# tjjones6/Computational-Fluid-Dynamics

Measured on AMD Instinct MI355X. Metric: Poisson MLUPS + steps/sec, cavity 4096² @1/2/4/8 GPU; % HBM roofline, higher is better.
Workload: dtype f64

## Files before the change

### computational-fluid-dynamics_amd/csrc/internal.hpp

```cpp
#pragma once

#include <stdexcept>
#include <string>
#include <vector>

#include "../../include/cfd_amd.h"

namespace cfd {

struct Error : std::runtime_error {
  int code;
  Error(int c, const std::string& m) : std::runtime_error(m), code(c) {}
};

void set_last_error(const std::string& msg);

struct LoopHub;
struct LoopOp {
  int kind;
  double* buf;
  size_t count;
  int peer;
};

// ... 1 lines not shown
  void* nccl = nullptr;
  int nranks = 1, rank = 0, device = 0;
  LoopHub* hub = nullptr;
  std::vector<LoopOp> pending;
  void* ev_ready = nullptr;
  void* ev_done = nullptr;
  double* tmp = nullptr;
  size_t tmp_count = 0;
};

void comm_unique_id(unsigned char* id_out);
Comm* comm_init(const unsigned char* id, int nranks, int rank, int device);
LoopHub* loop_hub_create(int nranks);
void loop_hub_destroy(LoopHub* h);
Comm* comm_init_loopback(LoopHub* h, int rank, int device);
void comm_destroy(Comm* c);
void comm_info(Comm* c, int* nranks, int* rank, int* transport);
void comm_group_start(Comm* c);
void comm_group_end(Comm* c, void* stream);
void comm_send(Comm* c, const double* buf, size_t count, int peer, void* stream);
void comm_recv(Comm* c, double* buf, size_t count, int peer, void* stream);
void comm_halo_exchange(Comm* c, const double* send_lo, double* recv_lo, int peer_lo, const double* send_hi,
                        double* recv_hi, int peer_hi, size_t count, void* stream);
long long comm_exchange_check(Comm* c, int peer, size_t count);
void comm_allreduce_max(Comm* c, double* buf, size_t count, void* stream);
void comm_allreduce_sum(Comm* c, double* buf, size_t count, void* stream);

void write_vtk_arrays(const cfd_params& p, const std::string& filename, double time_value, const double* uc,
                      const double* vc, const double* pr, const double* temp = nullptr);
void write_pvd(const std::string& filename, const char* const* files, const double* times, int n);

bool host_is_fluid(const cfd_params& p, int j, int i);

}
```

### computational-fluid-dynamics_amd/csrc/lexw.hpp

```cpp
#pragma once

#include "kernels.hpp"

namespace cfd {

constexpr int LEXW_SHARDS = 8;
#ifndef CFD_LEXW_RAMP_EDGE_FULL
#define CFD_LEXW_RAMP_EDGE_FULL 1
#endif
#ifndef CFD_LEXW_W2
#define CFD_LEXW_W2 2
#endif
#ifndef CFD_LEXW_W3
#define CFD_LEXW_W3 2
#endif
#define CFD_LEXW_MIN_WAVES(NS) ((NS) <= 2 ? CFD_LEXW_W2 : CFD_LEXW_W3)

__host__ __device__ constexpr int lexw_twc(int ns) { return ns >= 5 ? 106 : ns == 4 ? 110 : PAIR_TWC; }
__host__ __device__ constexpr int lexw_ch(int ns) { return ns >= 5 ? 10 : 8; }

constexpr int LEXW_RAMP_BANDS = 256;
struct LexRamp {
  int nb, th, row0;
  int wsplit;
  int xa, xn, xreach;
  unsigned band[LEXW_RAMP_BANDS];
};

__host__ __device__ inline int lexw_ramp_waves(const LexRamp& rp, int ctiles, int b, int ca, int cb, int o,
                                               int* ctile, int* half) {
  int sp[4], n = 0;
  if (rp.wsplit && ca == 0 && cb >= ca) sp[n++] = 0;
  if (rp.xn > 0 && rp.row0 + (b + 1) * rp.th + rp.xreach >= 0)
    for (int c = max(rp.xa, ca); c <= min(rp.xa + rp.xn - 1, cb); ++c)
      if (c != 0 && c != ctiles - 1) sp[n++] = c;
  if (rp.wsplit && cb == ctiles - 1 && cb > 0) sp[n++] = cb;
  int extra = 0;
  for (int q = 0; q < n; ++q) {
    const int at = sp[q] - ca + extra;
    if (o < at) break;
    if (o == at || o == at + 1) {
      *ctile = sp[q];
      *half = o - at;
      return n;
    }
    ++extra;
  }
  *ctile = ca + o - extra;
  *half = -1;
  return n;
}

// ... 21 lines not shown
}
__global__ void lexw_bits_scatter_kernel(LexCtl L, int ka, int kb, const double* __restrict__ flags) {
  const int k = ka + (int)(blockIdx.x * blockDim.x + threadIdx.x);
  if (k > kb || !(flags[k - ka] > 0.0)) return;
  const int q = L.kmax + k;
  atomicOr(L.bits + (q >> 6), 1ull << (q & 63));
}

__device__ __forceinline__ bool lexw_go_on(const LexCtl& L, int ka, int kb, bool first_wave, int lane) {
  if (L.stop[0] != 0) return false;
  const double tol = L.tol[0];
  for (int k = ka; k <= kb; ++k) {
    const bool go = (k == 0) ? (L.tol[1] > tol) : lexw_slot_exceeds(L, k);
    if (!go) {
      if (first_wave && lane == 0) {
        L.stop[1] = k;
        L.stop[0] = (k == 0 || k >= L.kexact) ? 1 : 2;
      }
      return false;
    }
  }
  return true;
}

#define LX_SLOT(X) ((((ROT) + 4 - (X)) % 5 + 10) % 5)
#define LX_S10(X) ((((6 * (ROT) + 5 * (PAR)) % 10 + 9 - (X)) % 10 + 20) % 10)


struct LxDefer {
  double xp, ps;
  int k;
};

template <int NS>
struct LexRun {
  double2 w[NS][5];
  double2 fr[10];
  double2 np[5];
  double2 nf[5];
  unsigned long long mask;
  LxDefer d;
};

struct LexCtx {
  int H0;
  int K;
  double tol;
  double o2, o3, o4;
  int jg, jr1;
  double gz;
};

__device__ __forceinline__ double2 lx_ld(const WaveCtx<CAVITY>& x, const double* base, int R) {
  const int Rc = min(max(R, x.rmin), x.rmax);
  return *reinterpret_cast<const double2*>(base + (size_t)(Rc - x.g.row_lo) * (size_t)x.g.pitch + x.gic);
}

constexpr int LX_ACT = 1;
#ifndef CFD_LEXW_GROUPS
#define CFD_LEXW_GROUPS 1
#endif
#ifndef CFD_LEXW_ALLRC
#define CFD_LEXW_ALLRC 0
#endif
constexpr int LX_SAMPLE = 2;
struct LxAct {
  bool a, b, c;
  bool a2, b2;
  unsigned u;
};
// ... 257 lines not shown
    if constexpr ((MODE & LX_ACT) != 0) ex = ex && act.c;
  } else {
    const double pc = m.x;
    double pW = dpp_from_left(old.y);
    if constexpr (STEP) pW = (rs == 2 && cc.sa == 2 && x.gi == x.c.step_i + 1) ? 0.0 + pc : pW;
    const double pS = row1 ? pc : sb.x;
    const double pE = m.y;
    ex = fabs(residual_at<CASE>(x.c, 0, 0, 0, 0, pc, pW, pE, pS, nb.x, fc.x)) > thr;
    if constexpr (EDGE) ex = ex && cc.ka == 3;
    if constexpr (STEP) {
      ex = ex && (rs == 0 || cc.sa == 2);
      if (rowc && cc.sa == 1) {
        ex = false;
        bool on = true;
        if constexpr ((MODE & LX_ACT) != 0) on = act.b;
        if (FULL && on) {
          d.xp = (pE - 2.0 * pc + pW) * x.c.idx2;
          d.ps = pS;
          d.k = (Hh - 1 - c0k) / 2 + 1;
          if (LASTH && x.out_lane && rrow) {
            L.cscr[0] = d.xp;
            L.cscr[1] = d.ps;
            L.cscr[2] = (double)d.k;
          }
        }
      }
    }
    if constexpr ((MODE & LX_ACT) != 0) ex = ex && act.b;
  }
  exi = ex ? 1 : exi;
  asm volatile("" : "+v"(exi));
}

template <int MODE, int T, int X>
constexpr bool lx_res_row() { return !(MODE & LX_SAMPLE) || T == X; }

template <int CASE>
struct LxCols {
  LxCol cc[2];
  LxoCol oc;
};

template <int CASE, int S, int NS, int T, int ROT, int PAR, int MODE, bool EDGE, bool RC, bool UP = false>
__device__ __forceinline__ void lx_sweeps(const WaveCtx<CAVITY>& x, const LexCtx& lc, const LexCtl& L,
                                          const LxCols<CASE>& cl, LexRun<NS>& s, int R, const LxAct& act, int& exi) {
  if constexpr (S < NS) {
    constexpr int D = UP ? -1 : 1;
    if constexpr (CASE == CAVITY) {
      lx_row<ROT, PAR ^ 1, 0, MODE, EDGE, false, lx_res_row<MODE, T, 2 * S + 1>(), UP>(
          x, lc, cl.cc, s.w[S], R + D * (2 * S + 1), 2 * S + 1, act, s.fr[LX_S10(2 * S + 1)], exi);
      lx_row<ROT, PAR, 1, MODE, EDGE, S == NS - 1, lx_res_row<MODE, T, 2 * S + 2>(), UP>(
          x, lc, cl.cc, s.w[S], R + D * (2 * S + 2), 2 * S + 2, act, s.fr[LX_S10(2 * S + 2)], exi);
    } else {
      lxo_row<CASE, ROT, PAR ^ 1, 0, MODE, EDGE, RC, false, lx_res_row<MODE, T, 2 * S + 1>(), S == 0, false, UP>(
          x, lc, L, cl.oc, s.w[S], R + D * (2 * S + 1), 2 * S + 1, act, s.fr[LX_S10(2 * S + 1)], exi, s.d);
      double2* nxt = nullptr;
      if constexpr (S + 1 < NS && !UP) nxt = &s.w[S + 1][LX_SLOT(2 * S + 3)];
      lxo_row<CASE, ROT, PAR, 1, MODE, EDGE, RC, S == NS - 1, lx_res_row<MODE, T, 2 * S + 2>(), false, S == NS - 1, UP>(
          x, lc, L, cl.oc, s.w[S], R + D * (2 * S + 2), 2 * S + 2, act, s.fr[LX_S10(2 * S + 2)], exi, s.d, nxt);
    }
    if constexpr (S + 1 < NS) s.w[S + 1][LX_SLOT(2 * S + 2)] = s.w[S][LX_SLOT(2 * S + 2)];
    lx_sweeps<CASE, S + 1, NS, T, ROT, PAR, MODE, EDGE, RC, UP>(x, lc, L, cl, s, R, act, exi);
  }
}

template <int CASE, int NS, int T, int ROT, int PAR, int MODE, bool EDGE, bool RC, bool UP = false>
__device__ __forceinline__ void lx_step(const WaveCtx<CAVITY>& x, const LexCtx& lc, const LexCtl& L,
                                        const LxCols<CASE>& cl, LexRun<NS>& s, int R, unsigned long long bit) {
  constexpr int D = UP ? -1 : 1;
  s.w[0][LX_SLOT(0)] = s.np[LX_SLOT(0)];
  s.fr[LX_S10(1)] = s.nf[LX_SLOT(0)];
  s.np[LX_SLOT(-4)] = lx_ld(x, x.pin, R - 4 * D);
  s.nf[LX_SLOT(-4)] = lx_ld(x, x.f, R - 3 * D);
  int exi = 0;
  const LxAct act = lx_act<MODE, CASE == BACKSTEP && EDGE && RC>(lc, x.gi, R);
  lx_sweeps<CASE, 0, NS, T, ROT, PAR, MODE, EDGE, RC, UP>(x, lc, L, cl, s, R, act, exi);
  if constexpr (UP) return;
  if constexpr ((MODE & LX_SAMPLE) && (T < 1 || T > 2 * NS)) return;
  s.mask |= exi ? bit : 0ull;
}

__device__ __forceinline__ unsigned long long wave_or64(unsigned long long v) {
#pragma unroll
  for (int off = 32; off > 0; off >>= 1) {
    const unsigned lo = (unsigned)v, hi = (unsigned)(v >> 32);
    v |= (unsigned long long)(unsigned)__shfl_xor((int)lo, off, 64) |
         ((unsigned long long)(unsigned)__shfl_xor((int)hi, off, 64) << 32);
  }
  return v;
}

__device__ __forceinline__ void lexw_flush(const LexCtl& L, int sh, int q0, const unsigned long long (&b)[3], int len) {
  unsigned long long* G = L.bits + (size_t)sh * L.words;
#pragma unroll
  for (int c = 0; c < 3; ++c) {
    if (c * 64 >= len || b[c] == 0) continue;
    const int q = q0 + c * 64;
    const int w = q >> 6, o = q & 63;
    if (w < L.words) atomicOr(&G[w], b[c] << o);
    if (o && w + 1 < L.words) atomicOr(&G[w + 1], b[c] >> (64 - o));
  }
}

template <int CASE, int NS, int MODE, bool EDGE, bool RC = false, bool UP = false>
__device__ __forceinline__ void lx_march(const WaveCtx<CAVITY>& x, const LexCtx& lc, const LexCtl& L, int y0, int y1,
                                         int c0, int lane, int shard) {
  static_assert(!UP || (!(MODE & LX_ACT) && !EDGE && !RC), "upward march: the unmasked, unchecked interior bands");
  constexpr int H = 2 * NS + 1;
  constexpr int D = UP ? -1 : 1;
  const int Rb0 = UP ? y0 - H : y1 - 1 + H;
  const int Rbeg = UP ? Rb0 - (Rb0 & 1) : Rb0 + (Rb0 & 1);
  const int nsteps = (y1 - y0) + 2 * H + (Rb0 & 1);
  LexRun<NS> s;
  const double2 z = make_double2(0.0, 0.0);
#pragma unroll
  for (int k = 0; k < 5; ++k)
#pragma unroll
    for (int q = 0; q < NS; ++q) s.w[q][k] = z;
#pragma unroll
  for (int k = 0; k < 10; ++k) s.fr[k] = z;
  {
    constexpr int ROT = 0;
#pragma unroll
    for (int q = 0; q < 4; ++q) {
      s.np[LX_SLOT(-q)] = lx_ld(x, x.pin, Rbeg - D * q);
      s.nf[LX_SLOT(-q)] = lx_ld(x, x.f, Rbeg - D * (q - 1));
    }
  }
  s.mask = 0ull;
  s.d = LxDefer{0.0, 0.0, -1};
  LxCols<CASE> cl;
  if constexpr (EDGE && CASE == CAVITY) cl.cc[0] = lx_col(x, x.gi), cl.cc[1] = lx_col(x, x.gi + 1);
  if constexpr (EDGE && CASE != CAVITY)
    cl.oc = LxoCol{lxo_kind(x, x.gi), lxo_kind(x, x.gi + 1), lxs_class(x, x.gi), lxs_class(x, x.gi + 1)};
  int R = Rbeg;
  if constexpr (UP) {
    for (int st = 0; st < nsteps; st += 10, R += 10) {
      lx_step<CASE, NS, 0, 0, 0, MODE, EDGE, RC, true>(x, lc, L, cl, s, R, 0ull);
      lx_step<CASE, NS, 1, 1, 1, MODE, EDGE, RC, true>(x, lc, L, cl, s, R + 1, 0ull);
      lx_step<CASE, NS, 2, 2, 0, MODE, EDGE, RC, true>(x, lc, L, cl, s, R + 2, 0ull);
      lx_step<CASE, NS, 3, 3, 1, MODE, EDGE, RC, true>(x, lc, L, cl, s, R + 3, 0ull);
      lx_step<CASE, NS, 4, 4, 0, MODE, EDGE, RC, true>(x, lc, L, cl, s, R + 4, 0ull);
      lx_step<CASE, NS, 5, 0, 1, MODE, EDGE, RC, true>(x, lc, L, cl, s, R + 5, 0ull);
      lx_step<CASE, NS, 6, 1, 0, MODE, EDGE, RC, true>(x, lc, L, cl, s, R + 6, 0ull);
      lx_step<CASE, NS, 7, 2, 1, MODE, EDGE, RC, true>(x, lc, L, cl, s, R + 7, 0ull);
      lx_step<CASE, NS, 8, 3, 0, MODE, EDGE, RC, true>(x, lc, L, cl, s, R + 8, 0ull);
      lx_step<CASE, NS, 9, 4, 1, MODE, EDGE, RC, true>(x, lc, L, cl, s, R + 9, 0ull);
    }
    return;
  }
#define LX_BIT(T) ((((st + (T)) >> 1) < 64) ? (1ull << ((st + (T)) >> 1)) : 0ull)
  for (int st = 0; st < nsteps; st += 10, R -= 10) {
#if CFD_LEXW_GROUPS
    if constexpr (RC && !EDGE && CASE == CHANNEL) {
      if (R - 8 >= 2 && R - 8 > x.rmin && R + 2 * NS < lc.jg && R + 2 * NS < x.rmax) {
        lx_step<CASE, NS, 0, 0, 0, MODE, EDGE, false>(x, lc, L, cl, s, R, LX_BIT(0));
        lx_step<CASE, NS, 1, 1, 1, MODE, EDGE, false>(x, lc, L, cl, s, R - 1, LX_BIT(1));
        lx_step<CASE, NS, 2, 2, 0, MODE, EDGE, false>(x, lc, L, cl, s, R - 2, LX_BIT(2));
        lx_step<CASE, NS, 3, 3, 1, MODE, EDGE, false>(x, lc, L, cl, s, R - 3, LX_BIT(3));
        lx_step<CASE, NS, 4, 4, 0, MODE, EDGE, false>(x, lc, L, cl, s, R - 4, LX_BIT(4));
        lx_step<CASE, NS, 5, 0, 1, MODE, EDGE, false>(x, lc, L, cl, s, R - 5, LX_BIT(5));
        lx_step<CASE, NS, 6, 1, 0, MODE, EDGE, false>(x, lc, L, cl, s, R - 6, LX_BIT(6));
        lx_step<CASE, NS, 7, 2, 1, MODE, EDGE, false>(x, lc, L, cl, s, R - 7, LX_BIT(7));
        lx_step<CASE, NS, 8, 3, 0, MODE, EDGE, false>(x, lc, L, cl, s, R - 8, LX_BIT(8));
        lx_step<CASE, NS, 9, 4, 1, MODE, EDGE, false>(x, lc, L, cl, s, R - 9, LX_BIT(9));
        continue;
      }
    }
#endif
    lx_step<CASE, NS, 0, 0, 0, MODE, EDGE, RC>(x, lc, L, cl, s, R, LX_BIT(0));
    lx_step<CASE, NS, 1, 1, 1, MODE, EDGE, RC>(x, lc, L, cl, s, R - 1, LX_BIT(1));
    lx_step<CASE, NS, 2, 2, 0, MODE, EDGE, RC>(x, lc, L, cl, s, R - 2, LX_BIT(2));
    lx_step<CASE, NS, 3, 3, 1, MODE, EDGE, RC>(x, lc, L, cl, s, R - 3, LX_BIT(3));
    lx_step<CASE, NS, 4, 4, 0, MODE, EDGE, RC>(x, lc, L, cl, s, R - 4, LX_BIT(4));
    lx_step<CASE, NS, 5, 0, 1, MODE, EDGE, RC>(x, lc, L, cl, s, R - 5, LX_BIT(5));
    lx_step<CASE, NS, 6, 1, 0, MODE, EDGE, RC>(x, lc, L, cl, s, R - 6, LX_BIT(6));
    lx_step<CASE, NS, 7, 2, 1, MODE, EDGE, RC>(x, lc, L, cl, s, R - 7, LX_BIT(7));
    lx_step<CASE, NS, 8, 3, 0, MODE, EDGE, RC>(x, lc, L, cl, s, R - 8, LX_BIT(8));
    lx_step<CASE, NS, 9, 4, 1, MODE, EDGE, RC>(x, lc, L, cl, s, R - 9, LX_BIT(9));
  }
#undef LX_BIT
  const unsigned long long m = x.out_lane ? s.mask : 0ull;
  const int sh = 63 - lane;
  const unsigned long long lo = m << sh, hi = sh ? (m >> (64 - sh)) : 0ull;
  unsigned long long b[3] = {wave_or64(lo), wave_or64(hi), 0ull};
  const int Bd0 = (lc.H0 - c0 - Rbeg - 2) / 2 + 1;
  if (lane == 0) lexw_flush(L, shard, Bd0 - 63 + L.kmax, b, 128);
}

__host__ __device__ inline void lexw_rows(const Geo& g, int H0, int K, int ns, int ct, int* lo, int* hi,
                                          bool open = false) {
  const int twc = lexw_twc(ns);
  if (!open) {
    const int cmin = max(ct * twc, 1), cmax = min(ct * twc + twc - 1, g.nx);
    *lo = max(g.j0, H0 - 2 * ns - 2 * (K - 1) - cmax);
    *hi = min(g.j1, H0 + 2 * ns - 1 - cmin);
  } else {
    const int cmin = max(ct * twc, 0), cmax = min(ct * twc + twc - 1, g.nx + 1);
    *lo = max(g.wj0, H0 - 2 * ns - 2 * (K - 1) - cmax - 2);
    *hi = min(g.wj1, H0 + 2 * ns - 1 - cmin);
  }
}

#ifndef CFD_LEXW_STAMPS
#define CFD_LEXW_STAMPS 0
#endif
#if CFD_LEXW_STAMPS
constexpr int LEXW_STAMP_LAUNCHES = 8192;
static __device__ unsigned long long lexw_stamp_buf[LEXW_STAMP_LAUNCHES * 8 * 3];
#ifndef LEXW_WSTAMP_L0
#define LEXW_WSTAMP_L0 1500
#endif
// ... 268 lines not shown
```

### computational-fluid-dynamics_amd/csrc/params.cpp

```cpp
#include <algorithm>
#include <cmath>
#include <cstring>
#include <string>

#include "internal.hpp"
#include "mg.hpp"

namespace {

double omega_2d(int nx, int ny) {
  const double pi = 3.14159265358979323846;
  const double rho_j = 0.5 * (std::cos(pi / (nx + 1)) + std::cos(pi / (ny + 1)));
  const double denom = 1.0 + std::sqrt(std::max(1e-14, 1.0 - rho_j * rho_j));
  return 2.0 / denom;
}

}

extern "C" int cfd_params_init(int case_id, double re, int nx, int ny, double dt, cfd_params* out) {
  if (!out) {
    cfd::set_last_error("null output");
    return CFD_E_ARG;
  }
  cfd_params p;
// ... 116 lines not shown

extern "C" int cfd_tuning_default(const cfd_params* p, int knob, int* value) {
  if (!p || !value) {
    cfd::set_last_error("null argument");
    return CFD_E_ARG;
  }
  const bool cav = p->case_id == CFD_CAVITY || p->case_id == CFD_RAYLEIGH_BENARD;
  switch (knob) {
    case CFD_TUNE_LEXW_EDGE_PCT: *value = p->ny <= 2048 ? 75 : 100; return CFD_OK;
    case CFD_TUNE_PAIR_EDGE_PCT: *value = cav ? 80 : 45; return CFD_OK;
    case CFD_TUNE_MARCH_MIN_TH: *value = (p->case_id == CFD_CHANNEL || p->ordering == CFD_ORDER_LEX) ? 16 : 24; return CFD_OK;
    case CFD_TUNE_TENT_TH: *value = 64; return CFD_OK;
    case CFD_TUNE_LEXW_RAMP_PCT:
      *value = p->case_id == CFD_BACKSTEP ? 100 : 0;
      return CFD_OK;
    case CFD_TUNE_TILE_ROUNDS: *value = cav ? 1 : 0; return CFD_OK;
    case CFD_TUNE_MARCH_ORDER: *value = 0; return CFD_OK;
    case CFD_TUNE_LEXW_LEFT: *value = 1; return CFD_OK;
    case CFD_TUNE_LEXW_UPDOWN: *value = 1; return CFD_OK;
    case CFD_TUNE_RESIDENT:
      *value = (cav || p->case_id == CFD_CHANNEL) ? 1 : 0;
      return CFD_OK;
    case CFD_TUNE_PAIR_WPS:
    case CFD_TUNE_WAVE_WPS:
    case CFD_TUNE_LEXW_WAVES:
      cfd::set_last_error("this knob's default is derived from the device's occupancy at cfd_create");
      return CFD_E_STATE;
    default:
      cfd::set_last_error("unknown tuning knob");
      return CFD_E_ARG;
  }
}

bool cfd::mg_make_plan(const cfd_params& p, MgPlan& plan, std::string& why) {
  if (p.case_id != CFD_CAVITY && p.case_id != CFD_RAYLEIGH_BENARD) {
    why = "multigrid covers the cavity and Rayleigh-Benard (case rule): the channel and the step keep SOR";
    return false;
  }
  if (p.nx < 2 || p.ny < 2 || !(p.dx > 0)) {
    why = "multigrid needs a grid of at least 2 x 2 cells and dx > 0 (grid rule)";
    return false;
  }
  int nx = p.nx, ny = p.ny, n = 0;
  plan = MgPlan{};
  for (;;) {
    MgLevel& L = plan.lv[n];
    L.nx = nx;
    L.ny = ny;
    L.pitch = ((nx + 3) + 15) / 16 * 16;
    L.lds_p = L.lds_f = -1;
    const int m = std::max(nx, ny);
    L.coarse_sweeps = 4 * m;
    L.h2 = std::ldexp(1.0, 2 * n) * (p.dx * p.dx);
    L.ih2 = 1.0 / L.h2;
    const double d = 0.5 + std::ldexp(1.0, -(n + 1));
    L.cS = 1.0 / d;
    L.g = 1.0 - L.cS;
    const double pi = 3.14159265358979323846;
    const double omega = 2.0 / (1.0 + std::sin(pi / (m + 1)));
    L.one_m_omega = 1.0 - omega;
    for (int k = 0; k < 16; ++k) {
      const double ew = k & 1, ee = (k >> 1) & 1, en = (k >> 2) & 1, cs = (k & 8) ? L.cS : 1.0;
      L.rdiag[k] = 1.0 / (((ew + ee) + en) + cs);
      L.omr[k] = omega * L.rdiag[k];
    }
    ++n;
// ... 51 lines not shown
```

### computational-fluid-dynamics_amd/csrc/solver.hip

```cpp
#include <algorithm>
#include <cmath>
#include <cstdlib>
#include <cstring>
#include <string>
#include <vector>

#include "internal.hpp"
#include "kernels.hpp"
#include "lexw.hpp"
#include "small.hpp"
#include "tile.hpp"
#include "resident.hpp"
#include "open.hpp"
#include "smlex.hpp"
#include "seqsum.hpp"
#include "mg.hpp"

#ifndef CFD_LEXW_WALL_SPLIT
#define CFD_LEXW_WALL_SPLIT 1
#endif

namespace cfd {

static thread_local std::string g_last_error;
// ... 180 lines not shown
      case CFD_TUNE_PAIR_WPS: resident_pair_waves = std::max(1, std::min(v, 4)) * 4 * n_cu; break;
      case CFD_TUNE_WAVE_WPS: resident_waves = std::max(1, std::min(v, 4)) * 4 * n_cu; break;
      case CFD_TUNE_LEXW_WAVES: resident_lexw_waves = std::max(64, v); break;
      case CFD_TUNE_LEXW_EDGE_PCT: lexw_edge_pct = std::max(10, std::min(100, v)); break;
      case CFD_TUNE_PAIR_EDGE_PCT: pair_edge_pct = std::max(10, std::min(100, v)); break;
      case CFD_TUNE_MARCH_MIN_TH: march_min_th = std::max(1, v); break;
      case CFD_TUNE_TENT_TH: tent_th = std::max(4, v); break;
      case CFD_TUNE_LEXW_RAMP_PCT: lexw_ramp_pct = std::max(0, std::min(100, v)); break;
      case CFD_TUNE_TILE_ROUNDS: tile_rounds = std::max(0, std::min(v, 16)); break;
      case CFD_TUNE_MARCH_ORDER: march_flags = (march_flags & ~8) | (v ? 8 : 0); break;
      case CFD_TUNE_LEXW_LEFT: lexw_left = v != 0; break;
      case CFD_TUNE_RESIDENT: res_knob = v != 0; break;
      case CFD_TUNE_LEXW_UPDOWN: lexw_updown = v != 0; break;
      default: throw Error(CFD_E_ARG, "unknown tuning knob");
    }
  }

  unsigned long long* lexbits = nullptr;
  size_t lexbits_words = 0;
  double* resmax = nullptr;
  hipEvent_t ev_f0 = nullptr, ev_f1 = nullptr;
  int resident_lexw_waves = 2048;
  int lexw_edge_pct = 100;
  int lexw_ramp_pct = 0;
  bool lexw_left = true;
  bool lexw_updown = true;
  bool step_lexw_ok() const { return P.step_i >= 2 && P.inlet_jmax >= 1 && P.inlet_jmax <= P.ny - 2; }
  bool use_lexw() const {
    return P.ordering == CFD_ORDER_LEX &&
           (P.case_id == CFD_CAVITY || P.case_id == CFD_CHANNEL || (P.case_id == CFD_BACKSTEP && step_lexw_ok()));
  }
  double* cscr = nullptr;
  int lexw_ns() const {
    const int ns = (P.case_id != CFD_CAVITY || P.sweeps_per_launch < 1) ? 4 : P.sweeps_per_launch;
    return multi() ? std::min(ns, 3) : ns;
  }
  bool ranks() const { return comm && comm->nranks > 1; }
  static constexpr int LEXW_RED_EVERY = 8;
  double* lexflags = nullptr;
  size_t lexflags_n = 0;
  void lexw_reduce_bits(const LexCtl& L, int ka, int kb) {
    if (!ranks() || ka > kb) return;
    const int n = kb - ka + 1;
    if ((size_t)n > lexflags_n) throw Error(CFD_E_STATE, "lexicographic ordering: bit reduction range");
    lexw_bits_gather_kernel<<<(n + 255) / 256, 256, 0, st>>>(L, ka, kb, lexflags);
    check_launch("lexw_bits_gather");
    comm_allreduce_max(comm, lexflags, (size_t)n, st);
    lexw_bits_scatter_kernel<<<(n + 255) / 256, 256, 0, st>>>(L, ka, kb, lexflags);
    check_launch("lexw_bits_scatter");
  }
  void seq_sum(const Strip& s, const double* a, const double* b, int mode, double* acc, bool accumulate) {
    T.seqsum_chunks += seq_sum_launch(s.g, C, a, b, mode, acc, accumulate ? 1 : 0, seqws, seqws_bytes, seqcnt, st);
    check_launch("seq_sum");
  }
  void flush_seq_count() {
    int n = 0;
    HIPC(hipMemcpyAsync(&n, seqcnt, sizeof(int), hipMemcpyDeviceToHost, st));
    HIPC(hipMemsetAsync(seqcnt, 0, sizeof(int), st));
    HIPC(hipStreamSynchronize(st));
    T.seqsum_serial_chunks += n;
  }
  void seq_sum_ranks(int a, int b, int mode, double* acc) {
    const int R = comm->nranks, me = comm->rank;
    const Strip& s = S[0];
    for (int q = 0; q < R; ++q) {
      if (q == me) seq_sum(s, s.b[a], b >= 0 ? s.b[b] : nullptr, mode, acc, me > 0);
      if (q + 1 < R) {
        comm_group_start(comm);
// ... 35 lines not shown
    }
    validate((int)rows.size());
    C = make_coef(P);
    proof_enabled = P.proof_test != CFD_OFF;
    proof_ns = P.sweeps_per_launch == 3 ? 3 : 4;
    HIPC(hipSetDevice(dev));
    hipDeviceProp_t prop;
    HIPC(hipGetDeviceProperties(&prop, dev));
    if (std::strncmp(prop.gcnArchName, "gfx950", 6) != 0)
      throw Error(CFD_E_DEVICE, std::string("libcfd_amd requires gfx950 (MI355X); device is ") + prop.gcnArchName);
    HIPC(hipStreamCreateWithFlags(&st, hipStreamNonBlocking));
    n_cu = prop.multiProcessorCount;
    {
      int wps = 0;
      HIPC(hipOccupancyMaxActiveBlocksPerMultiprocessor(&wps, poisson_wave_kernel<CAVITY>, 256, 0));
      wps = std::max(1, std::min(wps, 4));
      resident_waves = wps * 4 * prop.multiProcessorCount;
      int pps = 0;
      if (P.case_id == CFD_CAVITY)
        HIPC(hipOccupancyMaxActiveBlocksPerMultiprocessor(&pps, poisson_multi_kernel<CAVITY, 3>, 256, 0));
      else if (P.case_id == CFD_CHANNEL)
        HIPC(hipOccupancyMaxActiveBlocksPerMultiprocessor(&pps, poisson_multi_kernel<CHANNEL, 2>, 256, 0));
      else
        HIPC(hipOccupancyMaxActiveBlocksPerMultiprocessor(&pps, poisson_multi_kernel<BACKSTEP, 2>, 256, 0));
      pps = std::max(1, std::min(pps, 4));
      for (int knob : {CFD_TUNE_LEXW_EDGE_PCT, CFD_TUNE_PAIR_EDGE_PCT, CFD_TUNE_MARCH_MIN_TH, CFD_TUNE_TENT_TH,
                       CFD_TUNE_LEXW_RAMP_PCT, CFD_TUNE_TILE_ROUNDS, CFD_TUNE_MARCH_ORDER, CFD_TUNE_LEXW_LEFT,
                       CFD_TUNE_RESIDENT, CFD_TUNE_LEXW_UPDOWN}) {
        int v = 0;
        if (cfd_tuning_default(&P, knob, &v) == CFD_OK) set_tuning_value(knob, v);
      }
      if (P.case_id == CFD_CAVITY && proof_ok()) pps = std::min(pps, 2);
      if (use_lexw()) {
        int lps = 0;
        if (P.case_id == CFD_CHANNEL)
          HIPC(hipOccupancyMaxActiveBlocksPerMultiprocessor(&lps, poisson_lexw_kernel<CHANNEL, 4, false, true>, 256, 0));
        else if (P.case_id == CFD_BACKSTEP)
          HIPC(hipOccupancyMaxActiveBlocksPerMultiprocessor(&lps, poisson_lexw_kernel<BACKSTEP, 4, false, true>, 256, 0));
        else if (lexw_ns() == 4)
          HIPC(hipOccupancyMaxActiveBlocksPerMultiprocessor(&lps, poisson_lexw_kernel<CAVITY, 4, false, true>, 256, 0));
        else if (lexw_ns() == 1)
          HIPC(hipOccupancyMaxActiveBlocksPerMultiprocessor(&lps, poisson_lexw_kernel<CAVITY, 1, false>, 256, 0));
        else if (lexw_ns() == 2)
          HIPC(hipOccupancyMaxActiveBlocksPerMultiprocessor(&lps, poisson_lexw_kernel<CAVITY, 2, false>, 256, 0));
        else
          HIPC(hipOccupancyMaxActiveBlocksPerMultiprocessor(&lps, poisson_lexw_kernel<CAVITY, 3, false, true>, 256, 0));
        resident_lexw_waves = std::max(1, std::min(lps, 4)) * 4 * prop.multiProcessorCount;
      }
      resident_pair_waves = pps * 4 * prop.multiProcessorCount;
    }
    pitch = ((P.nx + 3) + 15) / 16 * 16;
    size_t part = 0;
    for (auto [j0, j1] : rows) {
      S.emplace_back();
      Strip& s = S.back();
      Geo& g = s.g;
      g.nx = P.nx;
      g.ny = P.ny;
      g.pitch = pitch;
      g.j0 = j0;
      g.j1 = j1;
      g.wj0 = (j0 == 1) ? 0 : j0;
      g.wj1 = (j1 == P.ny) ? P.ny + 1 : j1;
      g.row_lo = j0 - HALO;
      g.nrows = (j1 - j0 + 1) + 2 * HALO;
      const size_t n = (size_t)g.nrows * (size_t)pitch;
      for (int k = 0; k < NB; ++k) {
        if ((k == B_T || k == B_T2) && !thermal) continue;
        HIPC(hipMalloc(&s.b[k], n * sizeof(double)));
        HIPC(hipMemsetAsync(s.b[k], 0, n * sizeof(double), st));
      }
      s.grid2d = dim3((P.nx + 2 + 63) / 64, (j1 - j0 + 1 + 3) / 4);
      s.part_off = part;
      part += (size_t)s.grid2d.x * s.grid2d.y;
    }
    npart = part;
    const size_t ringn = (size_t)RING * RES_SHARDS * SHARD_STRIDE;
    HIPC(hipMalloc(&ring, ringn * sizeof(double)));
    HIPC(hipMalloc(&srcmax, RES_SHARDS * SHARD_STRIDE * sizeof(double)));
// ... 113 lines not shown
    res_bits = nullptr;
    res_bits_n = 0;
    lexbits_words = 0;
    if (stop) (void)hipFree(stop);
    stop = nullptr;
    if (h_stat) (void)hipHostFree(h_stat);
    if (h_shard) (void)hipHostFree(h_shard);
    h_stat = nullptr;
    h_shard = nullptr;
    for (auto& e : ev_poll)
      if (e) (void)hipEventDestroy(e);
    for (hipEvent_t e : {ev_a, ev_b, ev_s0, ev_s1, ev_f0, ev_f1})
      if (e) (void)hipEventDestroy(e);
    for (int q = 0; q < 2; ++q) {
      if (ev_int[q]) (void)hipEventDestroy(ev_int[q]);
      if (ev_bnd[q]) (void)hipEventDestroy(ev_bnd[q]);
    }
    if (ev_sync) (void)hipEventDestroy(ev_sync);
    if (st_b) (void)hipStreamDestroy(st_b);
    if (st) (void)hipStreamDestroy(st);
    ev_poll[0] = ev_poll[1] = ev_a = ev_b = ev_s0 = ev_s1 = ev_f0 = ev_f1 = ev_sync = nullptr;
    ev_int[0] = ev_int[1] = ev_bnd[0] = ev_bnd[1] = nullptr;
    st = st_b = nullptr;
  }

  void validate(int nstrips) const {
    if (P.case_id < 0 || P.case_id > 2) throw Error(CFD_E_ARG, "unknown case_id");
    if (P.nx < 2 || P.ny < 2) throw Error(CFD_E_ARG, "grid must have at least 2 interior cells per direction");
    if (!(P.dx > 0) || !(P.dy > 0) || !(P.dt > 0) || !(P.nu > 0) || !(P.rho > 0))
      throw Error(CFD_E_ARG, "dx, dy, dt, nu and rho must be positive");
    if (!(P.omega > 0) || !(P.omega < 2)) throw Error(CFD_E_ARG, "SOR omega must lie in (0, 2)");
    if (P.max_iters < 0) throw Error(CFD_E_ARG, "max_iters must be >= 0");
    if (P.check_every < 1) throw Error(CFD_E_ARG, "check_every must be >= 1");
    if (P.sweeps_per_launch < 0 || P.sweeps_per_launch > 5 ||
        (P.sweeps_per_launch == 5 && !(P.ordering == CFD_ORDER_LEX && P.case_id == CFD_CAVITY)))
      throw Error(CFD_E_ARG, "sweeps_per_launch must be 0 (auto), 1, 2, 3, 4 or 5 (the cavity's lexicographic order)");
    if (P.sweeps_per_launch == 3 && P.case_id != CFD_CAVITY && P.ordering == CFD_ORDER_RB)
      throw Error(CFD_E_ARG, "three red-black sweeps per launch are implemented for the cavity only");
    if (P.sweeps_per_launch >= 1 && P.sweeps_per_launch != 4 && P.ordering == CFD_ORDER_LEX &&
        P.case_id != CFD_CAVITY && P.case_id != CFD_RAYLEIGH_BENARD)
      throw Error(CFD_E_ARG, "the open cases' lexicographic-order kernel runs 4 sweeps per launch (0: auto)");
    if (P.sweeps_per_launch == 4 && P.ordering == CFD_ORDER_RB && P.proof_test == CFD_OFF)
      throw Error(CFD_E_ARG, "four red-black sweeps per launch need the proof-mode test (proof_test != CFD_OFF)");
    for (int sw : {P.proof_test, P.small_solve, P.overlap})
      if (sw < CFD_AUTO || sw > CFD_OFF) throw Error(CFD_E_ARG, "proof_test / small_solve / overlap must be a cfd_switch");
    if (P.ordering != CFD_ORDER_RB && P.ordering != CFD_ORDER_LEX) throw Error(CFD_E_ARG, "unknown ordering");
    if (P.ordering == CFD_ORDER_LEX && P.case_id == CFD_BACKSTEP && !step_lexw_ok() && (P.nx + P.ny) / 3 + 8 >= LEX_WIN)
      throw Error(CFD_E_ARG, "lexicographic ordering of a backwards step with a block under 2 cells wide or high "
                             "supports nx + ny < 12000");
    if (P.ordering == CFD_ORDER_LEX && P.case_id == CFD_BACKSTEP && !step_lexw_ok() && (nstrips > 1 || comm))
      throw Error(CFD_E_ARG, "lexicographic ordering of a backwards step with a block under 2 cells wide or high "
                             "runs on one strip (n_strips = 1, no ranks)");
#if CFD_WT_STORE
    if ((double)(P.ny + 2 * HALO + 2) * (double)(((P.nx + 3) + 15) / 16 * 16) * 8.0 >= 4294967295.0)
      throw Error(CFD_E_ARG, "the CFD_WT_STORE build addresses p buffers below 4 GiB: grid too large");
#endif
    if (P.case_id == CFD_BACKSTEP && (P.step_i <= 0 || P.step_i >= P.nx))
      throw Error(CFD_E_ARG, "Step location is outside computational domain!");
    if (P.case_id == CFD_BACKSTEP && (P.inlet_jmax < 1 || P.inlet_jmax > P.ny))
      throw Error(CFD_E_ARG, "inlet height is outside computational domain");
  }

  bool multi() const { return S.size() > 1 || comm != nullptr; }

  void exchange(int b, int depth, hipStream_t xs = nullptr) {
    if (!xs) xs = st;
    if (S.size() > 1) {
      for (size_t k = 0; k + 1 < S.size(); ++k) {
        Strip& lo = S[k];
// ... 475 lines not shown
    PairPlan plx = pl;
    if (steady && P.case_id == CFD_BACKSTEP && CFD_LEXW_XSPLIT > 1 && pl.nb1 == 0 && pl.ctiles >= 3) {
      const int jb = C.inlet_jmax + 1;
      int xa, xn;
      lexw_cross_tiles(ns, pl, &xa, &xn);
      int xb = -1;
      for (int b = 0; b < pl.nb0 && xb < 0; ++b)
        if (std::min(pl.lo0 + (b + 1) * pl.th, pl.hi0) + 4 * ns + 4 >= jb) xb = b;
      if (xa >= 0 && xb >= 0) {
        plx.xa = xa;
        plx.xn = xn;
        plx.xb = xb;
        plx.xbn = pl.nb0 - xb;
        plx.xparts = CFD_LEXW_XSPLIT;
        ntiles += plx.xn * plx.xbn * (plx.xparts - 1);
      }
    }
    if (ntiles == 0) return;
    const dim3 grid((ntiles + 3) / 4);
#define CFD_LEXW_LAUNCH(CASE, NS, R, SM) \
  poisson_lexw_kernel<CASE, NS, R, SM><<<grid, 256, 0, st>>>(g, C, pin, pout, f, L, H0, K, ka, kb, plx, fl, rp)
    if (P.case_id == CFD_BACKSTEP && ns == 3) {
      if (sample) { if (steady) CFD_LEXW_LAUNCH(BACKSTEP, 3, false, true); else CFD_LEXW_LAUNCH(BACKSTEP, 3, true, true); }
      else { if (steady) CFD_LEXW_LAUNCH(BACKSTEP, 3, false, false); else CFD_LEXW_LAUNCH(BACKSTEP, 3, true, false); }
    } else if (P.case_id == CFD_BACKSTEP) {
      if (sample) { if (steady) CFD_LEXW_LAUNCH(BACKSTEP, 4, false, true); else CFD_LEXW_LAUNCH(BACKSTEP, 4, true, true); }
      else { if (steady) CFD_LEXW_LAUNCH(BACKSTEP, 4, false, false); else CFD_LEXW_LAUNCH(BACKSTEP, 4, true, false); }
    } else if (P.case_id == CFD_CHANNEL && ns == 3) {
      if (sample) { if (steady) CFD_LEXW_LAUNCH(CHANNEL, 3, false, true); else CFD_LEXW_LAUNCH(CHANNEL, 3, true, true); }
      else { if (steady) CFD_LEXW_LAUNCH(CHANNEL, 3, false, false); else CFD_LEXW_LAUNCH(CHANNEL, 3, true, false); }
    } else if (P.case_id == CFD_CHANNEL) {
      if (sample) { if (steady) CFD_LEXW_LAUNCH(CHANNEL, 4, false, true); else CFD_LEXW_LAUNCH(CHANNEL, 4, true, true); }
      else { if (steady) CFD_LEXW_LAUNCH(CHANNEL, 4, false, false); else CFD_LEXW_LAUNCH(CHANNEL, 4, true, false); }
    } else if (ns == 5) {
      if (sample) { if (steady) CFD_LEXW_LAUNCH(CAVITY, 5, false, true); else CFD_LEXW_LAUNCH(CAVITY, 5, true, true); }
      else { if (steady) CFD_LEXW_LAUNCH(CAVITY, 5, false, false); else CFD_LEXW_LAUNCH(CAVITY, 5, true, false); }
    } else if (ns == 4) {
      if (sample) { if (steady) CFD_LEXW_LAUNCH(CAVITY, 4, false, true); else CFD_LEXW_LAUNCH(CAVITY, 4, true, true); }
      else { if (steady) CFD_LEXW_LAUNCH(CAVITY, 4, false, false); else CFD_LEXW_LAUNCH(CAVITY, 4, true, false); }
    } else if (ns == 1) { if (steady) CFD_LEXW_LAUNCH(CAVITY, 1, false, false); else CFD_LEXW_LAUNCH(CAVITY, 1, true, false); }
    else if (ns == 2) { if (steady) CFD_LEXW_LAUNCH(CAVITY, 2, false, false); else CFD_LEXW_LAUNCH(CAVITY, 2, true, false); }
    else if (sample) { if (steady) CFD_LEXW_LAUNCH(CAVITY, 3, false, true); else CFD_LEXW_LAUNCH(CAVITY, 3, true, true); }
    else { if (steady) CFD_LEXW_LAUNCH(CAVITY, 3, false, false); else CFD_LEXW_LAUNCH(CAVITY, 3, true, false); }
#undef CFD_LEXW_LAUNCH
  }

  int run_lexw(int base, int K, bool tests, int kexact, int ka0, int* kstop, int* code, bool time_steady) {
    const int ns = lexw_ns();
    const int Hlast = P.nx + P.ny + 2 * (K - 1) + (P.case_id != CFD_CAVITY ? 1 : 0);
    const int nl = (Hlast - 2) / (2 * ns) + 1;
    const int kmax = lexw_offset();
    LexCtl L{lexbits, (int)(lexbits_words / LEXW_SHARDS), kmax, tolv, stop, kexact, cscr};
    const int m_full = (!tests || kexact >= K) ? INT32_MAX : (ns >= 3) ? (2 * kexact - 1) / (2 * ns) : 0;
    std::vector<PairPlan> plans(S.size());
    for (size_t q = 0; q < S.size(); ++q)
      plans[q] = multi_plan(S[q].g.wj0, S[q].g.wj1 + 1, 0, 0, resident_lexw_waves / (int)S.size(), ns,
                            ns >= 5 ? 90 : 96,
                            lexw_edge_pct, lexw_twc(ns), lexw_extra(ns));
    std::vector<int> qs0(S.size()), qs1(S.size());
    int ms0 = 0, ms1 = INT32_MAX;
    for (size_t q = 0; q < S.size(); ++q) {
      const Geo& g = S[q].g;
      const int smax = P.nx + std::min(P.ny, g.j1 + HALO), smin = 1 + std::max(1, g.j0 - HALO);
      qs0[q] = (smax - 1 + 2 * ns - 1) / (2 * ns);
      qs1[q] = floordiv(smin + 2 * K - 2 * ns - 3, 2 * ns);
      ms0 = std::max(ms0, qs0[q]);
// ... 1477 lines not shown
```

Before: 751,100.

## Keep lexicographic RHS ring in LDS for deep cavity sweeps, add six-sweep variant

For the cavity lexicographic wavefront kernel with five or more fused sweeps, the per-lane ring of right-hand-side values moves from registers into a shared-memory ring, with one-ahead prefetch of the next sweep's values. This frees registers so more sweeps fit per launch. A six-sweep variant is added, auto-selection picks five sweeps for grids of 4096² and larger, and occupancy is now queried across both kernel instantiations. The cost is extra LDS traffic and shared memory per block, plus a longer pipeline ramp for deeper sweep counts.

```diff
diff --git a/computational-fluid-dynamics_amd/csrc/internal.hpp b/computational-fluid-dynamics_amd/csrc/internal.hpp
--- a/computational-fluid-dynamics_amd/csrc/internal.hpp
+++ b/computational-fluid-dynamics_amd/csrc/internal.hpp
@@ -57,4 +57,6 @@
 
 bool host_is_fluid(const cfd_params& p, int j, int i);
 
+int lexw_auto_sweeps(const cfd_params& p);
+
 }
diff --git a/computational-fluid-dynamics_amd/csrc/lexw.hpp b/computational-fluid-dynamics_amd/csrc/lexw.hpp
--- a/computational-fluid-dynamics_amd/csrc/lexw.hpp
+++ b/computational-fluid-dynamics_amd/csrc/lexw.hpp
@@ -16,8 +16,21 @@
 #endif
 #define CFD_LEXW_MIN_WAVES(NS) ((NS) <= 2 ? CFD_LEXW_W2 : CFD_LEXW_W3)
 
-__host__ __device__ constexpr int lexw_twc(int ns) { return ns >= 5 ? 106 : ns == 4 ? 110 : PAIR_TWC; }
-__host__ __device__ constexpr int lexw_ch(int ns) { return ns >= 5 ? 10 : 8; }
+__host__ __device__ constexpr int lexw_twc(int ns) {
+  return ns >= 6 ? 102 : ns == 5 ? 106 : ns == 4 ? 110 : PAIR_TWC;
+}
+__host__ __device__ constexpr int lexw_ch(int ns) { return ns >= 6 ? 12 : ns == 5 ? 10 : 8; }
+
+#ifndef CFD_LEXW_LDS4
+#define CFD_LEXW_LDS4 0
+#endif
+#ifndef CFD_LEXW_LDS_AHEAD
+#define CFD_LEXW_LDS_AHEAD 1
+#endif
+__host__ __device__ constexpr bool lexw_lds(int kcase, int ns) {
+  return kcase == CAVITY && (ns >= 5 || (ns == 4 && CFD_LEXW_LDS4));
+}
+__host__ __device__ constexpr int lexw_ring(int ns) { return ns <= 4 ? 8 : 16; }
 
 constexpr int LEXW_RAMP_BANDS = 256;
 struct LexRamp {
@@ -105,10 +118,12 @@
   int k;
 };
 
-template <int NS>
+template <int NS, bool LR = false>
 struct LexRun {
   double2 w[NS][5];
-  double2 fr[10];
+  double2 fr[LR ? 1 : 10];
+  double2* ring;
+  int rb;
   double2 np[5];
   double2 nf[5];
   unsigned long long mask;
@@ -432,8 +447,12 @@
   asm volatile("" : "+v"(exi));
 }
 
-template <int MODE, int T, int X>
-constexpr bool lx_res_row() { return !(MODE & LX_SAMPLE) || T == X; }
+template <int MODE, int T, int X, int NS>
+constexpr bool lx_res_row() {
+  return !(MODE & LX_SAMPLE) || (NS >= 5 ? (X - T + 2 * NS - 8 + 20) % 10 == 0 : T == X);
+}
+template <int MODE, int T, int NS>
+constexpr bool lx_res_step() { return !(MODE & LX_SAMPLE) || NS >= 5 || (T >= 1 && T <= 2 * NS); }
 
 template <int CASE>
 struct LxCols {
@@ -441,42 +460,62 @@
   LxoCol oc;
 };
 
-template <int CASE, int S, int NS, int T, int ROT, int PAR, int MODE, bool EDGE, bool RC, bool UP = false>
+template <int T, int ROT, int PAR, int X, int NS, bool LR>
+__device__ __forceinline__ double2 lx_fr(const LexRun<NS, LR>& s) {
+  if constexpr (LR) {
+    constexpr int D = lexw_ring(NS);
+    return s.ring[((s.rb + (T + 9 - X + D)) & (D - 1)) * 64];
+  } else {
+    return s.fr[LX_S10(X)];
+  }
+}
+
+template <int CASE, int S, int NS, int T, int ROT, int PAR, int MODE, bool EDGE, bool RC, bool UP = false, bool LR = false>
 __device__ __forceinline__ void lx_sweeps(const WaveCtx<CAVITY>& x, const LexCtx& lc, const LexCtl& L,
-                                          const LxCols<CASE>& cl, LexRun<NS>& s, int R, const LxAct& act, int& exi) {
+                                          const LxCols<CASE>& cl, LexRun<NS, LR>& s, int R, const LxAct& act, int& exi,
+                                          double2 f1 = make_double2(0.0, 0.0), double2 f2 = make_double2(0.0, 0.0)) {
   if constexpr (S < NS) {
+    constexpr bool AH = LR && CFD_LEXW_LDS_AHEAD;
+    if constexpr (!AH || S == 0) f1 = lx_fr<T, ROT, PAR, 2 * S + 1>(s), f2 = lx_fr<T, ROT, PAR, 2 * S + 2>(s);
+    double2 g1 = f1, g2 = f2;
+    if constexpr (AH && S + 1 < NS) g1 = lx_fr<T, ROT, PAR, 2 * S + 3>(s), g2 = lx_fr<T, ROT, PAR, 2 * S + 4>(s);
     constexpr int D = UP ? -1 : 1;
     if constexpr (CASE == CAVITY) {
-      lx_row<ROT, PAR ^ 1, 0, MODE, EDGE, false, lx_res_row<MODE, T, 2 * S + 1>(), UP>(
-          x, lc, cl.cc, s.w[S], R + D * (2 * S + 1), 2 * S + 1, act, s.fr[LX_S10(2 * S + 1)], exi);
-      lx_row<ROT, PAR, 1, MODE, EDGE, S == NS - 1, lx_res_row<MODE, T, 2 * S + 2>(), UP>(
-          x, lc, cl.cc, s.w[S], R + D * (2 * S + 2), 2 * S + 2, act, s.fr[LX_S10(2 * S + 2)], exi);
+      lx_row<ROT, PAR ^ 1, 0, MODE, EDGE, false, lx_res_row<MODE, T, 2 * S + 1, NS>(), UP>(
+          x, lc, cl.cc, s.w[S], R + D * (2 * S + 1), 2 * S + 1, act, f1, exi);
+      lx_row<ROT, PAR, 1, MODE, EDGE, S == NS - 1, lx_res_row<MODE, T, 2 * S + 2, NS>(), UP>(
+          x, lc, cl.cc, s.w[S], R + D * (2 * S + 2), 2 * S + 2, act, f2, exi);
     } else {
-      lxo_row<CASE, ROT, PAR ^ 1, 0, MODE, EDGE, RC, false, lx_res_row<MODE, T, 2 * S + 1>(), S == 0, false, UP>(
-          x, lc, L, cl.oc, s.w[S], R + D * (2 * S + 1), 2 * S + 1, act, s.fr[LX_S10(2 * S + 1)], exi, s.d);
+      lxo_row<CASE, ROT, PAR ^ 1, 0, MODE, EDGE, RC, false, lx_res_row<MODE, T, 2 * S + 1, NS>(), S == 0, false, UP>(
+          x, lc, L, cl.oc, s.w[S], R + D * (2 * S + 1), 2 * S + 1, act, f1, exi, s.d);
       double2* nxt = nullptr;
       if constexpr (S + 1 < NS && !UP) nxt = &s.w[S + 1][LX_SLOT(2 * S + 3)];
-      lxo_row<CASE, ROT, PAR, 1, MODE, EDGE, RC, S == NS - 1, lx_res_row<MODE, T, 2 * S + 2>(), false, S == NS - 1, UP>(
-          x, lc, L, cl.oc, s.w[S], R + D * (2 * S + 2), 2 * S + 2, act, s.fr[LX_S10(2 * S + 2)], exi, s.d, nxt);
+      lxo_row<CASE, ROT, PAR, 1, MODE, EDGE, RC, S == NS - 1, lx_res_row<MODE, T, 2 * S + 2, NS>(), false, S == NS - 1, UP>(
+          x, lc, L, cl.oc, s.w[S], R + D * (2 * S + 2), 2 * S + 2, act, f2, exi, s.d, nxt);
     }
     if constexpr (S + 1 < NS) s.w[S + 1][LX_SLOT(2 * S + 2)] = s.w[S][LX_SLOT(2 * S + 2)];
-    lx_sweeps<CASE, S + 1, NS, T, ROT, PAR, MODE, EDGE, RC, UP>(x, lc, L, cl, s, R, act, exi);
-  }
-}
-
-template <int CASE, int NS, int T, int ROT, int PAR, int MODE, bool EDGE, bool RC, bool UP = false>
+    lx_sweeps<CASE, S + 1, NS, T, ROT, PAR, MODE, EDGE, RC, UP, LR>(x, lc, L, cl, s, R, act, exi, g1, g2);
+  }
+}
+
+template <int CASE, int NS, int T, int ROT, int PAR, int MODE, bool EDGE, bool RC, bool UP = false, bool LR = false>
 __device__ __forceinline__ void lx_step(const WaveCtx<CAVITY>& x, const LexCtx& lc, const LexCtl& L,
-                                        const LxCols<CASE>& cl, LexRun<NS>& s, int R, unsigned long long bit) {
+                                        const LxCols<CASE>& cl, LexRun<NS, LR>& s, int R, unsigned long long bit) {
   constexpr int D = UP ? -1 : 1;
   s.w[0][LX_SLOT(0)] = s.np[LX_SLOT(0)];
-  s.fr[LX_S10(1)] = s.nf[LX_SLOT(0)];
+  if constexpr (LR) {
+    constexpr int RD = lexw_ring(NS);
+    s.ring[((s.rb + (T + 8 + RD)) & (RD - 1)) * 64] = s.nf[LX_SLOT(0)];
+  } else {
+    s.fr[LX_S10(1)] = s.nf[LX_SLOT(0)];
+  }
   s.np[LX_SLOT(-4)] = lx_ld(x, x.pin, R - 4 * D);
   s.nf[LX_SLOT(-4)] = lx_ld(x, x.f, R - 3 * D);
   int exi = 0;
   const LxAct act = lx_act<MODE, CASE == BACKSTEP && EDGE && RC>(lc, x.gi, R);
-  lx_sweeps<CASE, 0, NS, T, ROT, PAR, MODE, EDGE, RC, UP>(x, lc, L, cl, s, R, act, exi);
+  lx_sweeps<CASE, 0, NS, T, ROT, PAR, MODE, EDGE, RC, UP, LR>(x, lc, L, cl, s, R, act, exi);
   if constexpr (UP) return;
-  if constexpr ((MODE & LX_SAMPLE) && (T < 1 || T > 2 * NS)) return;
+  if constexpr (!lx_res_step<MODE, T, NS>()) return;
   s.mask |= exi ? bit : 0ull;
 }
 
@@ -502,6 +541,12 @@
   }
 }
 
+template <int NS>
+__device__ __forceinline__ double2* lx_ring() {
+  __shared__ double2 ring[4 * lexw_ring(NS) * 64];
+  return ring;
+}
+
 template <int CASE, int NS, int MODE, bool EDGE, bool RC = false, bool UP = false>
 __device__ __forceinline__ void lx_march(const WaveCtx<CAVITY>& x, const LexCtx& lc, const LexCtl& L, int y0, int y1,
                                          int c0, int lane, int shard) {
@@ -511,14 +556,22 @@
   const int Rb0 = UP ? y0 - H : y1 - 1 + H;
   const int Rbeg = UP ? Rb0 - (Rb0 & 1) : Rb0 + (Rb0 & 1);
   const int nsteps = (y1 - y0) + 2 * H + (Rb0 & 1);
-  LexRun<NS> s;
+  constexpr bool LR = lexw_lds(CASE, NS);
+  LexRun<NS, LR> s;
   const double2 z = make_double2(0.0, 0.0);
 #pragma unroll
   for (int k = 0; k < 5; ++k)
 #pragma unroll
     for (int q = 0; q < NS; ++q) s.w[q][k] = z;
+  if constexpr (LR) {
+    s.ring = lx_ring<NS>() + (threadIdx.x >> 6) * (lexw_ring(NS) * 64) + lane;
+    s.rb = 0;
 #pragma unroll
-  for (int k = 0; k < 10; ++k) s.fr[k] = z;
+    for (int k = 0; k < lexw_ring(NS); ++k) s.ring[k * 64] = z;
+  } else {
+#pragma unroll
+    for (int k = 0; k < 10; ++k) s.fr[k] = z;
+  }
   {
     constexpr int ROT = 0;
 #pragma unroll
@@ -546,6 +599,7 @@
       lx_step<CASE, NS, 7, 2, 1, MODE, EDGE, RC, true>(x, lc, L, cl, s, R + 7, 0ull);
       lx_step<CASE, NS, 8, 3, 0, MODE, EDGE, RC, true>(x, lc, L, cl, s, R + 8, 0ull);
       lx_step<CASE, NS, 9, 4, 1, MODE, EDGE, RC, true>(x, lc, L, cl, s, R + 9, 0ull);
+      if constexpr (LR) s.rb = (s.rb + 10) & (lexw_ring(NS) - 1);
     }
     return;
   }
@@ -578,6 +632,7 @@
     lx_step<CASE, NS, 7, 2, 1, MODE, EDGE, RC>(x, lc, L, cl, s, R - 7, LX_BIT(7));
     lx_step<CASE, NS, 8, 3, 0, MODE, EDGE, RC>(x, lc, L, cl, s, R - 8, LX_BIT(8));
     lx_step<CASE, NS, 9, 4, 1, MODE, EDGE, RC>(x, lc, L, cl, s, R - 9, LX_BIT(9));
+    if constexpr (LR) s.rb = (s.rb + 10) & (lexw_ring(NS) - 1);
   }
 #undef LX_BIT
   const unsigned long long m = x.out_lane ? s.mask : 0ull;
diff --git a/computational-fluid-dynamics_amd/csrc/params.cpp b/computational-fluid-dynamics_amd/csrc/params.cpp
--- a/computational-fluid-dynamics_amd/csrc/params.cpp
+++ b/computational-fluid-dynamics_amd/csrc/params.cpp
@@ -172,6 +172,11 @@
   }
 }
 
+int cfd::lexw_auto_sweeps(const cfd_params& p) {
+  const bool cav = p.case_id == CFD_CAVITY || p.case_id == CFD_RAYLEIGH_BENARD;
+  return (cav && (long long)p.nx * p.ny >= 4096LL * 4096LL) ? 5 : 4;
+}
+
 bool cfd::mg_make_plan(const cfd_params& p, MgPlan& plan, std::string& why) {
   if (p.case_id != CFD_CAVITY && p.case_id != CFD_RAYLEIGH_BENARD) {
     why = "multigrid covers the cavity and Rayleigh-Benard (case rule): the channel and the step keep SOR";
diff --git a/computational-fluid-dynamics_amd/csrc/solver.hip b/computational-fluid-dynamics_amd/csrc/solver.hip
--- a/computational-fluid-dynamics_amd/csrc/solver.hip
+++ b/computational-fluid-dynamics_amd/csrc/solver.hip
@@ -236,8 +236,15 @@
   }
   double* cscr = nullptr;
   int lexw_ns() const {
-    const int ns = (P.case_id != CFD_CAVITY || P.sweeps_per_launch < 1) ? 4 : P.sweeps_per_launch;
+    const int ns = P.case_id != CFD_CAVITY ? 4 : P.sweeps_per_launch < 1 ? lexw_auto_sweeps(P) : P.sweeps_per_launch;
     return multi() ? std::min(ns, 3) : ns;
+  }
+  template <int CASE, int NS, bool SAMPLE>
+  static int lexw_blocks() {
+    int a = 0, b = 0;
+    HIPC(hipOccupancyMaxActiveBlocksPerMultiprocessor(&a, poisson_lexw_kernel<CASE, NS, false, SAMPLE>, 256, 0));
+    HIPC(hipOccupancyMaxActiveBlocksPerMultiprocessor(&b, poisson_lexw_kernel<CASE, NS, true, SAMPLE>, 256, 0));
+    return std::min(a, b);
   }
   bool ranks() const { return comm && comm->nranks > 1; }
   static constexpr int LEXW_RED_EVERY = 8;
@@ -339,19 +346,16 @@
       }
       if (P.case_id == CFD_CAVITY && proof_ok()) pps = std::min(pps, 2);
       if (use_lexw()) {
+        const int ns = lexw_ns();
         int lps = 0;
-        if (P.case_id == CFD_CHANNEL)
-          HIPC(hipOccupancyMaxActiveBlocksPerMultiprocessor(&lps, poisson_lexw_kernel<CHANNEL, 4, false, true>, 256, 0));
-        else if (P.case_id == CFD_BACKSTEP)
-          HIPC(hipOccupancyMaxActiveBlocksPerMultiprocessor(&lps, poisson_lexw_kernel<BACKSTEP, 4, false, true>, 256, 0));
-        else if (lexw_ns() == 4)
-          HIPC(hipOccupancyMaxActiveBlocksPerMultiprocessor(&lps, poisson_lexw_kernel<CAVITY, 4, false, true>, 256, 0));
-        else if (lexw_ns() == 1)
-          HIPC(hipOccupancyMaxActiveBlocksPerMultiprocessor(&lps, poisson_lexw_kernel<CAVITY, 1, false>, 256, 0));
-        else if (lexw_ns() == 2)
-          HIPC(hipOccupancyMaxActiveBlocksPerMultiprocessor(&lps, poisson_lexw_kernel<CAVITY, 2, false>, 256, 0));
-        else
-          HIPC(hipOccupancyMaxActiveBlocksPerMultiprocessor(&lps, poisson_lexw_kernel<CAVITY, 3, false, true>, 256, 0));
+        if (P.case_id == CFD_CHANNEL) lps = ns == 3 ? lexw_blocks<CHANNEL, 3, true>() : lexw_blocks<CHANNEL, 4, true>();
+        else if (P.case_id == CFD_BACKSTEP) lps = ns == 3 ? lexw_blocks<BACKSTEP, 3, true>() : lexw_blocks<BACKSTEP, 4, true>();
+        else if (ns == 6) lps = lexw_blocks<CAVITY, 6, true>();
+        else if (ns == 5) lps = lexw_blocks<CAVITY, 5, true>();
+        else if (ns == 4) lps = lexw_blocks<CAVITY, 4, true>();
+        else if (ns == 1) lps = lexw_blocks<CAVITY, 1, false>();
+        else if (ns == 2) lps = lexw_blocks<CAVITY, 2, false>();
+        else lps = lexw_blocks<CAVITY, 3, true>();
         resident_lexw_waves = std::max(1, std::min(lps, 4)) * 4 * prop.multiProcessorCount;
       }
       resident_pair_waves = pps * 4 * prop.multiProcessorCount;
@@ -531,9 +535,18 @@
     if (!(P.omega > 0) || !(P.omega < 2)) throw Error(CFD_E_ARG, "SOR omega must lie in (0, 2)");
     if (P.max_iters < 0) throw Error(CFD_E_ARG, "max_iters must be >= 0");
     if (P.check_every < 1) throw Error(CFD_E_ARG, "check_every must be >= 1");
-    if (P.sweeps_per_launch < 0 || P.sweeps_per_launch > 5 ||
-        (P.sweeps_per_launch == 5 && !(P.ordering == CFD_ORDER_LEX && P.case_id == CFD_CAVITY)))
-      throw Error(CFD_E_ARG, "sweeps_per_launch must be 0 (auto), 1, 2, 3, 4 or 5 (the cavity's lexicographic order)");
+    if (P.sweeps_per_launch < 0 || P.sweeps_per_launch > 6 ||
+        (P.sweeps_per_launch >= 5 && !(P.ordering == CFD_ORDER_LEX && P.case_id == CFD_CAVITY)))
+      throw Error(CFD_E_ARG,
+                  "sweeps_per_launch must be 0 (auto), 1, 2, 3, 4 or 5, 6 (the cavity's lexicographic order)");
+    if (P.sweeps_per_launch == 6 && P.small_solve != CFD_OFF && nstrips == 1 && !comm) {
+      Geo g{};
+      g.nx = P.nx;
+      g.ny = P.ny;
+      if (smlex_fits(g, make_coef(P)))
+        throw Error(CFD_E_ARG, "sweeps_per_launch 6 runs in the multi-block reference-order march: this grid goes to "
+                               "the one-workgroup solve (small_solve off selects the march)");
+    }
     if (P.sweeps_per_launch == 3 && P.case_id != CFD_CAVITY && P.ordering == CFD_ORDER_RB)
       throw Error(CFD_E_ARG, "three red-black sweeps per launch are implemented for the cavity only");
     if (P.sweeps_per_launch >= 1 && P.sweeps_per_launch != 4 && P.ordering == CFD_ORDER_LEX &&
@@ -1075,6 +1088,9 @@
     } else if (P.case_id == CFD_CHANNEL) {
       if (sample) { if (steady) CFD_LEXW_LAUNCH(CHANNEL, 4, false, true); else CFD_LEXW_LAUNCH(CHANNEL, 4, true, true); }
       else { if (steady) CFD_LEXW_LAUNCH(CHANNEL, 4, false, false); else CFD_LEXW_LAUNCH(CHANNEL, 4, true, false); }
+    } else if (ns == 6) {
+      if (sample) { if (steady) CFD_LEXW_LAUNCH(CAVITY, 6, false, true); else CFD_LEXW_LAUNCH(CAVITY, 6, true, true); }
+      else { if (steady) CFD_LEXW_LAUNCH(CAVITY, 6, false, false); else CFD_LEXW_LAUNCH(CAVITY, 6, true, false); }
     } else if (ns == 5) {
       if (sample) { if (steady) CFD_LEXW_LAUNCH(CAVITY, 5, false, true); else CFD_LEXW_LAUNCH(CAVITY, 5, true, true); }
       else { if (steady) CFD_LEXW_LAUNCH(CAVITY, 5, false, false); else CFD_LEXW_LAUNCH(CAVITY, 5, true, false); }
```

After: 792,000, median of 6. 5.4% higher.
